# telespazio-tim/karios

Measured on AMD Instinct MI355X. Metric: Mpixels/sec (+ matched keypoints/sec), Sentinel-2 10980^2 pair, KLT + ZNCC, higher is better.
Workload: dtype u8/i32 stencils, f32 LK solve, f64 stretch + ZNCC; 1 GPU; BASELINE config 2: 4 distinct S2-sized pairs 10980x10980 u16 resident in HBM, one per step, 4 per batched submissio...; distinct_pairs_resident=4, contexts=1, klt=Laplacian k=7, maxCorners 20000, one tile, ZNCC of rows with score >= 0.4, parallelism=1 rank(s), each a stream of independent band pairs

## Files before the change

karios_amd/csrc/k_eig3.hip:

```cpp
#include <cstring>
#include <string.h>

#include "eig2_item.hpp"

namespace {

#define EIG3_STAGE 1024
#define EIG3_FLUSH_AT 384
#define EIG3_SEG 3
#define EIG3_MARGIN 12
#define EIG3_STRIDE (512 - 2 * EIG3_MARGIN)

__device__ __forceinline__ int e3_mad_lo(uint32_t a, uint32_t b, int c)
{
    int d;
    asm("v_mad_i32_i16 %0, %1, %2, %3" : "=v"(d) : "v"(a), "v"(b), "v"(c));
    return d;
}
__device__ __forceinline__ int e3_mad_hi(uint32_t a, uint32_t b, int c)
{
    int d;
    asm("v_mad_i32_i16 %0, %1, %2, %3 op_sel:[1,1,0,0]" : "=v"(d) : "v"(a), "v"(b), "v"(c));
    return d;
}
__device__ __forceinline__ uint32_t e3_pk_mad2(uint32_t a, uint32_t c)
{
    uint32_t d;
    asm("v_pk_mad_u16 %0, %1, %2, %3" : "=v"(d) : "v"(a), "s"(0x00020002u), "v"(c));
    return d;
}
__device__ __forceinline__ int e3_add_next(int w, int v)
{
    int d;
    asm("v_add_u32_dpp %0, %1, %2 wave_shl:1 row_mask:0xf bank_mask:0xf bound_ctrl:1" : "=v"(d) : "v"(v), "v"(w));
    return d;
}
__device__ __forceinline__ int e3_add_prev(int w, int v)
{
    int d;
    asm("v_add_u32_dpp %0, %1, %2 wave_shr:1 row_mask:0xf bank_mask:0xf bound_ctrl:1" : "=v"(d) : "v"(v), "v"(w));
    return d;
}
__device__ __forceinline__ int e3_next_minus(int v, int w)
{
    int d;
    asm("v_sub_u32_dpp %0, %1, %2 wave_shl:1 row_mask:0xf bank_mask:0xf bound_ctrl:1" : "=v"(d) : "v"(v), "v"(w));
    return d;
}
__device__ __forceinline__ int e3_prev_minus(int v, int w)
{
    int d;
    asm("v_sub_u32_dpp %0, %1, %2 wave_shr:1 row_mask:0xf bank_mask:0xf bound_ctrl:1" : "=v"(d) : "v"(v), "v"(w));
    return d;
}

template <class F, int... I> __device__ __forceinline__ void e3_for_impl(F &&f, std::integer_sequence<int, I...>)
{
    (f(std::integral_constant<int, I>{}), ...);
}
template <int N, class F> __device__ __forceinline__ void e3_for(F &&f) { e3_for_impl(f, std::make_integer_sequence<int, N>{}); }

template <int BLOCK>
__device__ __forceinline__ void eig3_item(const uint8_t *__restrict__ src, const uint8_t *__restrict__ mask, int H, int W, double scale2,
                                          unsigned *__restrict__ max_partial, double quality, km_scalars *sc, unsigned long long *__restrict__ keys,
                                          size_t cap, unsigned stage_cap, int wave_id, int xs, int col_lo, int col_hi, int ye0, int ye1,
                                          unsigned long long *st , int count_skips = 0)
{
    constexpr int L = BLOCK / 2, Rr = BLOCK - 1 - L;
    static_assert(L <= 7 && Rr <= 7, "the box window must stay within the two neighbouring lanes");
    const int lane = threadIdx.x & 63;
    const int c0 = xs + 8 * lane;
    const int m_first = ye0 - L, m_last = ye1 + Rr;

    uint32_t colmask[2] = {0u, 0u};
#pragma unroll
    for (int p = 0; p < 8; p++)
        if (c0 + p >= col_lo && c0 + p < col_hi) colmask[p >> 2] |= 0xffu << (8 * (p & 3));
    const uint8_t *mptr = mask ? mask : src;
    const uint32_t mask_or = mask ? 0u : 0x01010101u;

    auto load8 = [&](const uint8_t *base, int r) -> uint2 {
        const uint8_t *rowp = base + (size_t)r * W;
        uint2 v;
        __builtin_memcpy(&v, rowp + e2_opaque((unsigned)c0), 8);
        return v;
    };
    struct row4 { uint32_t q[4]; };
    auto unpack = [&](uint2 w) -> row4 {
        row4 r;
        r.q[0] = __builtin_amdgcn_perm(0u, w.x, 0x0c010c00u);
        r.q[1] = __builtin_amdgcn_perm(0u, w.x, 0x0c030c02u);
        r.q[2] = __builtin_amdgcn_perm(0u, w.y, 0x0c010c00u);
        r.q[3] = __builtin_amdgcn_perm(0u, w.y, 0x0c030c02u);
        return r;
    };
    auto derivs = [&](const row4 &r0, const row4 &r1, const row4 &r2, uint32_t (&dx)[4], uint32_t (&dy)[4]) {
        uint32_t t0[4], t1[4], m0[5], m1[5];
#pragma unroll
        for (int i = 0; i < 4; i++) {
            t0[i] = e3_pk_mad2(r1.q[i], e2u(e2s(r0.q[i]) + e2s(r2.q[i])));
            t1[i] = e2u(e2s(r2.q[i]) - e2s(r0.q[i]));
        }
        asm("s_nop 1" : "+v"(t0[0]), "+v"(t0[3]));
        const uint32_t l0 = (uint32_t)e2_lane_m1((int)t0[3]), r0n = (uint32_t)e2_lane_p1((int)t0[0]);
        const uint32_t l1 = (uint32_t)e2_lane_m1((int)t1[3]), r1n = (uint32_t)e2_lane_p1((int)t1[0]);
#pragma unroll
        for (int i = 0; i < 5; i++) {
            const uint32_t lo0 = i == 0 ? l0 : t0[i - 1], hi0 = i == 4 ? r0n : t0[i];
            const uint32_t lo1 = i == 0 ? l1 : t1[i - 1], hi1 = i == 4 ? r1n : t1[i];
            m0[i] = __builtin_amdgcn_alignbyte(hi0, lo0, 2);
            m1[i] = __builtin_amdgcn_alignbyte(hi1, lo1, 2);
        }
#pragma unroll
        for (int i = 0; i < 4; i++) {
            dx[i] = e2u(e2s(m0[i + 1]) - e2s(m0[i]));
            dy[i] = e2u(e2s(e3_pk_mad2(t1[i], m1[i])) + e2s(m1[i + 1]));
        }
    };
    int V[3][8];
#pragma unroll
    for (int q = 0; q < 3; q++)
#pragma unroll
        for (int p = 0; p < 8; p++) V[q][p] = 0;
    auto accumulate = [&](const uint32_t (&dx)[4], const uint32_t (&dy)[4], bool subtract) {
#pragma unroll
        for (int i = 0; i < 4; i++) {
            const uint32_t x = dx[i], y = dy[i];
            const uint32_t sx = subtract ? e2u(-e2s(x)) : x, sy = subtract ? e2u(-e2s(y)) : y;
            V[0][2 * i] = e3_mad_lo(x, sx, V[0][2 * i]);
            V[0][2 * i + 1] = e3_mad_hi(x, sx, V[0][2 * i + 1]);
            V[1][2 * i] = e3_mad_lo(x, sy, V[1][2 * i]);
            V[1][2 * i + 1] = e3_mad_hi(x, sy, V[1][2 * i + 1]);
            V[2][2 * i] = e3_mad_lo(y, sy, V[2][2 * i]);
            V[2][2 * i + 1] = e3_mad_hi(y, sy, V[2][2 * i + 1]);
        }
    };
    auto windows = [&](auto &&emit ) {
        auto add_ext = [&](int w, auto q_tag, auto kt) -> int {
            constexpr int q = decltype(q_tag)::value, k = decltype(kt)::value;
            if constexpr (k < 0) return e3_add_prev(w, V[q][k + 8]);
            else if constexpr (k > 7) return e3_add_next(w, V[q][k - 8]);
            else return w + V[q][k];
        };
        auto ext_minus = [&](auto q_tag, auto kt, int w) -> int {
            constexpr int q = decltype(q_tag)::value, k = decltype(kt)::value;
            if constexpr (k < 0) return e3_prev_minus(V[q][k + 8], w);
            else if constexpr (k > 7) return e3_next_minus(V[q][k - 8], w);
            else return V[q][k] - w;
        };
        int w[3];
        e3_for<3>([&](auto qt) {
            constexpr int q = decltype(qt)::value;
            if constexpr (L == 7 && Rr == 7) {
                const int T = ((V[q][0] + V[q][1]) + (V[q][2] + V[q][3])) + ((V[q][4] + V[q][5]) + (V[q][6] + V[q][7]));
                w[q] = T + e2_lane_m1(T - V[q][0]);
            } else {
                w[q] = 0;
                e3_for<BLOCK>([&](auto kt) { w[q] = add_ext(w[q], qt, std::integral_constant<int, decltype(kt)::value - L>{}); });
            }
        });
        emit(std::integral_constant<int, 0>{}, w[0], w[1], w[2]);
        e3_for<7>([&](auto pt) {
            constexpr int P = decltype(pt)::value;
            int t[3];
            e3_for<3>([&](auto qt) { t[decltype(qt)::value] = ext_minus(qt, std::integral_constant<int, P - L>{}, w[decltype(qt)::value]); });
            e3_for<3>([&](auto qt) {
                constexpr int q = decltype(qt)::value;
                w[q] = ext_minus(qt, std::integral_constant<int, P + 1 + Rr>{}, t[q]);
            });
            emit(std::integral_constant<int, P + 1>{}, w[0], w[1], w[2]);
        });
    };
    const double scale2h = scale2 * 0.5;
    auto lambda_min = [&](int sxx, int sxy, int syy) {
        const float a = (float)__dmul_rn((double)sxx, scale2h);
        const float b = (float)__dmul_rn((double)sxy, scale2);
        const float cc = (float)__dmul_rn((double)syy, scale2h);
        const float t = __fsub_rn(a, cc);
        const float sq = __fadd_rn(__fmul_rn(t, t), __fmul_rn(b, b));
        return __fsub_rn(__fadd_rn(a, cc), e2_sqrt(sq));
    };

    float best = -INFINITY;
    unsigned tie_rows = 0u;
#ifdef KM_DEV
    unsigned skip_total = 0u, skip_hit = 0u;
#endif
    unsigned cnt = 0;
    const unsigned shard = (unsigned)wave_id % KM_NSHARD;
    const size_t cap_s = cap / KM_NSHARD;
    auto flush_if = [&](unsigned threshold) {
        if (cnt <= threshold) return;
        if (cnt > stage_cap) { if (lane == 0) atomicOr(&sc->pad0, 1u); cnt = min(cnt, (unsigned)EIG3_STAGE); }
        unsigned base = 0;
        if (lane == 0) base = atomicAdd(&sc->shard_cnt[shard], cnt);
        base = __shfl(base, 0);
        for (unsigned i = lane; i < cnt; i += 64)
            if ((size_t)base + i < cap_s) keys[shard * cap_s + base + i] = st[i];
        cnt = 0;
    };
    float thr_run = 0.f;
    unsigned published = 0u, gk_seen = 0u;
    auto refresh_threshold = [&](bool global) {
        unsigned wk = best > -INFINITY ? e2_key(best) : 0u;
        for (int o = 32; o > 0; o >>= 1) wk = max(wk, (unsigned)__shfl_xor((int)wk, o));
        if (global) {
            gk_seen = __hip_atomic_load(&sc->run_max_shard[wave_id & 63], __ATOMIC_RELAXED, __HIP_MEMORY_SCOPE_AGENT);
        } else if (published == 0u && wk > gk_seen && (gk_seen == 0u || e2_unkey(wk) > e2_unkey(gk_seen) * 1.0625f)) {
            if (lane == 0) atomicMax(&sc->run_max_shard[wave_id & 63], wk);
            published = 1u;
        }
        const unsigned mk2 = max(wk, gk_seen);
        thr_run = mk2 ? (float)__dmul_rn((double)e2_unkey(mk2), quality) : 0.f;
    };

    row4 LW[3], TW[3];
    float E[3][8];
    float EM[8];
#pragma unroll
    for (int k = 0; k < 3; k++)
#pragma unroll
        for (int p = 0; p < 8; p++) E[k][p] = 0.f;
#pragma unroll
    for (int p = 0; p < 8; p++) EM[p] = -INFINITY;

    auto compute = [&](auto ph_tag, int m, uint2 mkraw, bool trail, bool out, bool cand) {
        constexpr int PH = decltype(ph_tag)::value;
        constexpr int S0 = PH, S1 = (PH + 1) % 3, S2 = (PH + 2) % 3;
        uint32_t dx[4], dy[4];
        derivs(LW[S0], LW[S1], LW[S2], dx, dy);
        accumulate(dx, dy, false);
        if (trail) {
            derivs(TW[S0], TW[S1], TW[S2], dx, dy);
            accumulate(dx, dy, true);
        }
        if (!out) return;
        const int y = m - Rr;
        constexpr int C = PH, P1 = (PH + 2) % 3, P2 = (PH + 1) % 3;
        {
            asm("s_nop 4" : "+v"(V[0][0]), "+v"(V[0][1]), "+v"(V[0][2]), "+v"(V[0][3]), "+v"(V[0][4]), "+v"(V[0][5]), "+v"(V[0][6]), "+v"(V[0][7]),
                            "+v"(V[1][0]), "+v"(V[1][1]), "+v"(V[1][2]), "+v"(V[1][3]), "+v"(V[1][4]), "+v"(V[1][5]), "+v"(V[1][6]), "+v"(V[1][7]),
                            "+v"(V[2][0]), "+v"(V[2][1]), "+v"(V[2][2]), "+v"(V[2][3]), "+v"(V[2][4]), "+v"(V[2][5]), "+v"(V[2][6]), "+v"(V[2][7]));
#ifdef KM_DEV
            if (count_skips) {
                windows([&](auto pt, int sxx, int sxy, int syy) {
                    E[C][decltype(pt)::value] = lambda_min(sxx, sxy, syy);
                    const float bound = (float)__dmul_rn((double)min(sxx, syy), scale2);
                    skip_total++;
                    skip_hit += __ballot(!(bound <= thr_run)) == 0ull ? 1u : 0u;
                });
            } else
#endif
            windows([&](auto pt, int sxx, int sxy, int syy) { E[C][decltype(pt)::value] = lambda_min(sxx, sxy, syy); });
        }
        if (cand) {
            float m3[8];
#pragma unroll
            for (int p = 0; p < 8; p++) m3[p] = fmaxf(fmaxf(E[P2][p], E[P1][p]), E[C][p]);
            const float m3l = __int_as_float(e2_lane_m1(__float_as_int(m3[7]))), m3r = __int_as_float(e2_lane_p1(__float_as_int(m3[0])));
            auto is_cand = [&](int p) {
                const float left = p == 0 ? m3l : m3[(p + 7) & 7], right = p == 7 ? m3r : m3[(p + 1) & 7];
                const float nb = fmaxf(fmaxf(left, right), m3[p]);
                return EM[p] > thr_run && EM[p] >= nb;
            };
            float selval = 0.f;
            unsigned selp = 0u, ncand = 0u;
            bool isv[8];
#pragma unroll
            for (int p = 0; p < 8; p++) {
                const bool is = isv[p] = is_cand(p);
                selval = is ? EM[p] : selval;
                selp = is ? (unsigned)p : selp;
                ncand += is ? 1u : 0u;
            }
            const unsigned rowidx = (unsigned)(y - 1) * (unsigned)W + (unsigned)c0;
            const unsigned long long multi = __ballot(ncand > 1u);
            auto append = [&](unsigned long long bal, bool mine, float v, unsigned p) {
                const unsigned slot = cnt + __builtin_amdgcn_mbcnt_hi((unsigned)(bal >> 32), __builtin_amdgcn_mbcnt_lo((unsigned)bal, 0u));
                st[min(mine ? slot : ~0u, EIG3_STAGE + (unsigned)lane)] = ((unsigned long long)__float_as_uint(v) << 32) | (unsigned long long)(rowidx + p);
                cnt += (unsigned)__popcll(bal);
            };
            if (__builtin_expect(multi == 0ull, 1)) {
                append(__ballot(ncand != 0u), ncand != 0u, selval, selp);
            } else if (__ballot(ncand > 2u) == 0ull) {
                float fval = selval;
                unsigned fp = selp;
#pragma unroll
                for (int p = 6; p >= 0; p--) {
                    fval = isv[p] ? EM[p] : fval;
                    fp = isv[p] ? (unsigned)p : fp;
                }
                append(__ballot(ncand != 0u), ncand != 0u, selval, selp);
                append(multi, ncand > 1u, fval, fp);
            } else {
                tie_rows++;
#pragma unroll
                for (int p = 0; p < 8; p++) {
                    const bool is = isv[p];
                    const unsigned long long bal = __ballot(is);
                    const unsigned slot = cnt + __builtin_amdgcn_mbcnt_hi((unsigned)(bal >> 32), __builtin_amdgcn_mbcnt_lo((unsigned)bal, 0u));
                    st[min(is ? slot : ~0u, EIG3_STAGE + (unsigned)lane)] =
                        ((unsigned long long)__float_as_uint(EM[p]) << 32) | (unsigned long long)(rowidx + (unsigned)p);
                    cnt += (unsigned)__popcll(bal);
                }
            }
        }
        const uint32_t mk[2] = {(mkraw.x | mask_or) & colmask[0], (mkraw.y | mask_or) & colmask[1]};
#pragma unroll
        for (int p = 0; p < 8; p++) {
            const bool counts = ((mk[p >> 2] >> (8 * (p & 3))) & 0xffu) != 0u;
            EM[p] = counts ? E[C][p] : -INFINITY;
            best = fmaxf(best, EM[p]);
        }
    };

    auto entering3 = [&](int m, row4 (&win)[3], auto ph_tag) {
        constexpr int PH = decltype(ph_tag)::value;
        const int r = km_reflect101(m, H);
        win[PH] = unpack(load8(src, km_reflect101(r - 1, H)));
        win[(PH + 1) % 3] = unpack(load8(src, r));
        win[(PH + 2) % 3] = unpack(load8(src, km_reflect101(r + 1, H)));
    };
    auto clamp_row = [&](int r) { return min(max(r, 0), H - 1); };
    auto general_step = [&](int m, auto ph_tag) {
        const int step = m - m_first;
        entering3(m, LW, ph_tag);
        const bool trail = step >= BLOCK;
        if (trail) entering3(m - BLOCK, TW, ph_tag);
        const bool out = step >= BLOCK - 1;
        const uint2 mkraw = load8(mptr, clamp_row(m - Rr));
        compute(ph_tag, m, mkraw, trail, out, out && (m - Rr) >= ye0 + 2);
    };
    int m = m_first;
    auto general_until = [&](int m_end, bool align3) {
        for (; m <= m_last; m++) {
            const int step = m - m_first;
            if (m > m_end && (!align3 || step % 3 == 0)) break;
            if ((step & 7) == 0) refresh_threshold(m == m_first);
            switch (step % 3) {
            case 0: general_step(m, std::integral_constant<int, 0>{}); break;
            case 1: general_step(m, std::integral_constant<int, 1>{}); break;
            default: general_step(m, std::integral_constant<int, 2>{}); break;
            }
            flush_if(EIG3_FLUSH_AT);
        }
    };
    const bool early = m_first >= 1 && BLOCK >= 5;
    const int mi_lo = early ? m_first + 1 : max(m_first + BLOCK + 1, BLOCK + 1), mi_hi = min(m_last, H - 2 - 3);
    general_until(min(mi_lo - 1, m_last), true);
    if (m <= mi_hi && m + 2 <= mi_hi) {
        uint2 ql[3], qt[3], qm[3];
#pragma unroll
        for (int k = 0; k < 3; k++) {
            ql[k] = load8(src, m + k + 1);
            qt[k] = load8(src, max(m + k - BLOCK + 1, 0));
            qm[k] = load8(mptr, max(m + k - Rr, 0));
        }
        while (m + 2 <= mi_hi && m - m_first < BLOCK + 1) {
            e3_for<3>([&](auto kt) {
                constexpr int K = decltype(kt)::value;
                const int step = m + K - m_first;
                LW[(K + 2) % 3] = unpack(ql[K]);
                TW[(K + 2) % 3] = unpack(qt[K]);
                compute(kt, m + K, qm[K], step >= BLOCK, step >= BLOCK - 1, step >= BLOCK - 1 && m + K - Rr >= ye0 + 2);
                ql[K] = load8(src, m + K + 3 + 1);
                qt[K] = load8(src, max(m + K + 3 - BLOCK + 1, 0));
                qm[K] = load8(mptr, max(m + K + 3 - Rr, 0));
            });
            m += 3;
        }
        while (m + 2 <= mi_hi) {
            flush_if(EIG3_FLUSH_AT);
            refresh_threshold(false);
            const int seg_end = min(mi_hi, m + EIG3_SEG * 3 - 1);
            for (; m + 2 <= seg_end; m += 3) {
                e3_for<3>([&](auto kt) {
                    constexpr int K = decltype(kt)::value;
                    LW[(K + 2) % 3] = unpack(ql[K]);
                    TW[(K + 2) % 3] = unpack(qt[K]);
                    compute(kt, m + K, qm[K], true, true, true);
                    ql[K] = load8(src, m + K + 3 + 1);
                    qt[K] = load8(src, m + K + 3 - BLOCK + 1);
                    qm[K] = load8(mptr, m + K + 3 - Rr);
                });
            }
        }
    }
    general_until(m_last, false);
    flush_if(0u);
    unsigned key = best > -INFINITY ? e2_key(best) : 0u;
    for (int o = 32; o > 0; o >>= 1) key = max(key, (unsigned)__shfl_xor((int)key, o));
    if (lane == 0) max_partial[wave_id] = key;
    if (lane == 0 && tie_rows) atomicAdd(&sc->tie_rows, tie_rows);
#ifdef KM_DEV
    if (lane == 0 && count_skips) { atomicAdd(&sc->skip_total, (unsigned long long)skip_total); atomicAdd(&sc->skip_hit, (unsigned long long)skip_hit); }
#endif
}

struct e3_units_args {
    const uint8_t *src[KM_UNITS_MAX], *mask[KM_UNITS_MAX];
    unsigned *max_partial[KM_UNITS_MAX];
    km_scalars *sc[KM_UNITS_MAX];
    unsigned long long *keys[KM_UNITS_MAX];
    int H[KM_UNITS_MAX], W[KM_UNITS_MAX], n_border[KM_UNITS_MAX], nstrips[KM_UNITS_MAX];
    int item0[KM_UNITS_MAX + 1];
    int n, rows2, rows3;
    int count_skips;
};
template <int BLOCK>
__global__ __launch_bounds__(256, 3) void eig3_units_kernel(e3_units_args U, double scale2, double quality, size_t cap, unsigned stage_cap2, unsigned stage_cap3)
{
    __shared__ int xs_scratch[4][3][128];
    __shared__ unsigned long long stage[4][EIG3_STAGE + 64];
    const int wv = __builtin_amdgcn_readfirstlane(threadIdx.x >> 6);
    const int total = U.item0[U.n];
    unsigned tile;
    if (!km_xcd_tile((unsigned)(total + 3) / 4u, tile)) return;
    const int wave_lin = (int)tile * 4 + wv;
    if (wave_lin >= total) return;
    int u = 0;
    while (u + 1 < U.n && wave_lin >= U.item0[u + 1]) u++;
    const int wave_id = wave_lin - U.item0[u];
    const uint8_t *src = U.src[u], *mask = U.mask[u];
    const int H = U.H[u], W = U.W[u], n_border = U.n_border[u], nstrips = U.nstrips[u];
    unsigned *max_partial = U.max_partial[u];
    km_scalars *sc = U.sc[u];
    unsigned long long *keys = U.keys[u];
    if (wave_id < n_border) {
        const int rowblock = wave_id >> 1;
        const bool right = wave_id & 1;
        constexpr int ML2 = eig2_geom<BLOCK, true>::ML;
        eig2_item<BLOCK, true>(src, mask, H, W, scale2, nullptr, max_partial, U.rows2, quality, sc, keys, cap, stage_cap2, wave_id, rowblock,
                               right ? W - EIG3_MARGIN - ML2 : -ML2, right ? W - EIG3_MARGIN : 0, right ? W : EIG3_MARGIN, &xs_scratch[wv][0][0], stage[wv]);
        return;
    }
    const int j = wave_id - n_border;
    const int rowblock = j / nstrips, strip = j - rowblock * nstrips;
    const int xs = min(strip * EIG3_STRIDE, W - 512);
    const int col_lo = EIG3_MARGIN + strip * EIG3_STRIDE, col_hi = min(col_lo + EIG3_STRIDE, W - EIG3_MARGIN);
    const int ye0 = rowblock * U.rows3, ye1 = min(H - 1, ye0 + U.rows3 + 1);
    eig3_item<BLOCK>(src, mask, H, W, scale2, max_partial, quality, sc, keys, cap, stage_cap3, wave_id, xs, col_lo, col_hi, ye0, ye1, stage[wv],
                     U.count_skips);
}

template <int BLOCK>
int launch_eig3_units(km_ctx *c, km_units &U, double scale2, double quality, bool single)
{
    e3_units_args A;
    A.n = U.n; A.rows2 = 64;
    long border_total = 0;
    for (int u = 0; u < U.n; u++) {
        A.src[u] = U.lap_ref[u]; A.mask[u] = U.mask[u]; A.sc[u] = U.sc[u]; A.keys[u] = U.keys[u];
        A.H[u] = U.H[u]; A.W[u] = U.W[u];
        A.nstrips[u] = (U.W[u] - 2 * EIG3_MARGIN + EIG3_STRIDE - 1) / EIG3_STRIDE;
        A.n_border[u] = 2 * ((U.H[u] - 2 + A.rows2 - 1) / A.rows2);
        border_total += A.n_border[u];
    }
    (void)border_total;
    int rows3 = 0;
    for (int u = 0; u < U.n; u++) {
        const int r = km_pick_rows(U.H[u] - 2, A.nstrips[u], 5, 1024L * 3 - A.n_border[u], 32, 192);
        rows3 = r > rows3 ? r : rows3;
    }
    if (!single) rows3 = std::min(std::max(rows3, 48), 96);
    if (const char *e = km_dev_env("KARIOS_HIP_EIG3_ROWS")) { const int v = atoi(e); if (v >= 8 && v <= 8192) rows3 = v; }
    A.rows3 = rows3;
    A.item0[0] = 0;
    for (int u = 0; u < U.n; u++) A.item0[u + 1] = A.item0[u] + A.n_border[u] + A.nstrips[u] * ((U.H[u] - 2 + rows3 - 1) / rows3);
    const int total = A.item0[U.n];
    unsigned *partial = (unsigned *)km_ws(c, WS_PARTIAL, ((size_t)total + 16) * sizeof(unsigned));
    if (!partial) return KM_E_NOMEM;
    for (int u = 0; u < U.n; u++) {
        A.max_partial[u] = partial + A.item0[u];
        U.eig_partial[u] = A.max_partial[u]; U.eig_npartial[u] = (unsigned)(A.item0[u + 1] - A.item0[u]);
    }
    const unsigned cap2 = c->opt_stage_cap > 0 && c->opt_stage_cap < EIG2_STAGE ? (unsigned)c->opt_stage_cap : (unsigned)EIG2_STAGE;
    const unsigned cap3 = c->opt_stage_cap > 0 && c->opt_stage_cap < EIG3_STAGE ? (unsigned)c->opt_stage_cap : (unsigned)EIG3_STAGE;
    A.count_skips = c->opt_eig3_count ? 1 : 0;
    eig3_units_kernel<BLOCK><<<km_xcd_grid((unsigned)(total + 3) / 4u), 256, 0, c->stream>>>(A, scale2, quality, U.capk, cap2, cap3);
    KM_LAUNCH_CHECK(c);
    return KM_OK;
}

__global__ __launch_bounds__(1024) void eig3_max_kernel(const unsigned *__restrict__ partial, unsigned n, unsigned *out)
{
    unsigned m = 0;
    for (unsigned i = threadIdx.x; i < n; i += 1024) m = max(m, partial[i]);
    for (int o = 32; o > 0; o >>= 1) m = max(m, (unsigned)__shfl_xor((int)m, o));
    __shared__ unsigned sh[16];
    if ((threadIdx.x & 63) == 0) sh[threadIdx.x >> 6] = m;
    __syncthreads();
    if (threadIdx.x == 0) {
        unsigned t = 0;
        for (int i = 0; i < 16; i++) t = max(t, sh[i]);
        *out = t;
    }
}

}

int k3_eig_candidates_units(km_ctx *c, km_units &U, int block, double quality)
{
    if (block < 1 || block > 15 || (block & 1) == 0 || !c->opt_eig3) return KM_E_UNSUPPORTED;
    for (int u = 0; u < U.n; u++)
        if (U.W[u] < 512 || U.H[u] < 2 * block + 8) return KM_E_UNSUPPORTED;
    const double scale = 1.0 / (4.0 * (double)block * 255.0), s2 = scale * scale;
    switch (block) {
#define KM_EIG3_CASE(B) case B: return launch_eig3_units<B>(c, U, s2, quality, false);
        KM_EIG3_CASE(1) KM_EIG3_CASE(3) KM_EIG3_CASE(5) KM_EIG3_CASE(7) KM_EIG3_CASE(9) KM_EIG3_CASE(11) KM_EIG3_CASE(13) KM_EIG3_CASE(15)
#undef KM_EIG3_CASE
    default: return KM_E_UNSUPPORTED;
    }
}

int k3_eig_candidates(km_ctx *c, const uint8_t *d_src, const uint8_t *d_mask, int H, int W, int block, double quality, km_scalars *sc,
                      unsigned long long *d_keys, size_t cap, km_eig_partials *partials)
{
    if (block < 1 || block > 15 || (block & 1) == 0) return KM_E_UNSUPPORTED;
    if (W < 512 || H < 2 * block + 8) return KM_E_UNSUPPORTED;
    const double scale = 1.0 / (4.0 * (double)block * 255.0), s2 = scale * scale;
    km_units U;
    U.n = 1; U.H[0] = H; U.W[0] = W; U.capk = cap;
    U.lap_ref[0] = const_cast<uint8_t *>(d_src); U.mask[0] = const_cast<uint8_t *>(d_mask); U.sc[0] = sc; U.keys[0] = d_keys;
    int rc;
    switch (block) {
#define KM_EIG3_CASE(B) case B: rc = launch_eig3_units<B>(c, U, s2, quality, true); break;
        KM_EIG3_CASE(1) KM_EIG3_CASE(3) KM_EIG3_CASE(5) KM_EIG3_CASE(7) KM_EIG3_CASE(9) KM_EIG3_CASE(11) KM_EIG3_CASE(13) KM_EIG3_CASE(15)
#undef KM_EIG3_CASE
    default: return KM_E_UNSUPPORTED;
    }
    if (rc) return rc;
    if (partials) {
        partials->partial = U.eig_partial[0]; partials->n = U.eig_npartial[0];
        return KM_OK;
    }
    eig3_max_kernel<<<1, 1024, 0, c->stream>>>(U.eig_partial[0], U.eig_npartial[0], &sc->max_eig_key);
    KM_LAUNCH_CHECK(c);
    return KM_OK;
}
```

Measured before the change: 160,100 Mpx/s.

## Pack leading and trailing rows into u16 pairs and accumulate with sdot2

Rows entering and leaving the sliding box window are now interleaved into one packed 16-bit pair per pixel, with the leading row in the low half and the trailing row in the high half. Derivatives for both rows are computed together, and a single v_dot2 with a sign vector (+1,-1) updates the structure-tensor sums. This replaces two separate derivative passes and pairs of mad_i32_i16 instructions, and removes the alignbyte shuffles because each pixel now sits in its own dword. The cost is twice as many registers per row window, and the pk_mad trick and 16-bit overflow behaviour now depend on the interleaving.

```diff
diff --git a/karios_amd/csrc/k_eig3.hip b/karios_amd/csrc/k_eig3.hip
--- a/karios_amd/csrc/k_eig3.hip
+++ b/karios_amd/csrc/k_eig3.hip
@@ -11,18 +11,7 @@
 #define EIG3_MARGIN 12
 #define EIG3_STRIDE (512 - 2 * EIG3_MARGIN)
 
-__device__ __forceinline__ int e3_mad_lo(uint32_t a, uint32_t b, int c)
-{
-    int d;
-    asm("v_mad_i32_i16 %0, %1, %2, %3" : "=v"(d) : "v"(a), "v"(b), "v"(c));
-    return d;
-}
-__device__ __forceinline__ int e3_mad_hi(uint32_t a, uint32_t b, int c)
-{
-    int d;
-    asm("v_mad_i32_i16 %0, %1, %2, %3 op_sel:[1,1,0,0]" : "=v"(d) : "v"(a), "v"(b), "v"(c));
-    return d;
-}
+__device__ __forceinline__ int e3_dot2(uint32_t a, uint32_t b, int c) { return __builtin_amdgcn_sdot2(e2s(a), e2s(b), c, false); }
 __device__ __forceinline__ uint32_t e3_pk_mad2(uint32_t a, uint32_t c)
 {
     uint32_t d;
@@ -85,36 +74,35 @@
         __builtin_memcpy(&v, rowp + e2_opaque((unsigned)c0), 8);
         return v;
     };
-    struct row4 { uint32_t q[4]; };
-    auto unpack = [&](uint2 w) -> row4 {
-        row4 r;
-        r.q[0] = __builtin_amdgcn_perm(0u, w.x, 0x0c010c00u);
-        r.q[1] = __builtin_amdgcn_perm(0u, w.x, 0x0c030c02u);
-        r.q[2] = __builtin_amdgcn_perm(0u, w.y, 0x0c010c00u);
-        r.q[3] = __builtin_amdgcn_perm(0u, w.y, 0x0c030c02u);
+    struct row8 { uint32_t d[8]; };
+    auto pack = [&](uint2 lead, uint2 trail) -> row8 {
+        row8 r;
+        r.d[0] = __builtin_amdgcn_perm(trail.x, lead.x, 0x0c040c00u);
+        r.d[1] = __builtin_amdgcn_perm(trail.x, lead.x, 0x0c050c01u);
+        r.d[2] = __builtin_amdgcn_perm(trail.x, lead.x, 0x0c060c02u);
+        r.d[3] = __builtin_amdgcn_perm(trail.x, lead.x, 0x0c070c03u);
+        r.d[4] = __builtin_amdgcn_perm(trail.y, lead.y, 0x0c040c00u);
+        r.d[5] = __builtin_amdgcn_perm(trail.y, lead.y, 0x0c050c01u);
+        r.d[6] = __builtin_amdgcn_perm(trail.y, lead.y, 0x0c060c02u);
+        r.d[7] = __builtin_amdgcn_perm(trail.y, lead.y, 0x0c070c03u);
         return r;
     };
-    auto derivs = [&](const row4 &r0, const row4 &r1, const row4 &r2, uint32_t (&dx)[4], uint32_t (&dy)[4]) {
-        uint32_t t0[4], t1[4], m0[5], m1[5];
-#pragma unroll
-        for (int i = 0; i < 4; i++) {
-            t0[i] = e3_pk_mad2(r1.q[i], e2u(e2s(r0.q[i]) + e2s(r2.q[i])));
-            t1[i] = e2u(e2s(r2.q[i]) - e2s(r0.q[i]));
-        }
-        asm("s_nop 1" : "+v"(t0[0]), "+v"(t0[3]));
-        const uint32_t l0 = (uint32_t)e2_lane_m1((int)t0[3]), r0n = (uint32_t)e2_lane_p1((int)t0[0]);
-        const uint32_t l1 = (uint32_t)e2_lane_m1((int)t1[3]), r1n = (uint32_t)e2_lane_p1((int)t1[0]);
-#pragma unroll
-        for (int i = 0; i < 5; i++) {
-            const uint32_t lo0 = i == 0 ? l0 : t0[i - 1], hi0 = i == 4 ? r0n : t0[i];
-            const uint32_t lo1 = i == 0 ? l1 : t1[i - 1], hi1 = i == 4 ? r1n : t1[i];
-            m0[i] = __builtin_amdgcn_alignbyte(hi0, lo0, 2);
-            m1[i] = __builtin_amdgcn_alignbyte(hi1, lo1, 2);
-        }
-#pragma unroll
-        for (int i = 0; i < 4; i++) {
-            dx[i] = e2u(e2s(m0[i + 1]) - e2s(m0[i]));
-            dy[i] = e2u(e2s(e3_pk_mad2(t1[i], m1[i])) + e2s(m1[i + 1]));
+    auto derivs = [&](const row8 &r0, const row8 &r1, const row8 &r2, uint32_t (&dx)[8], uint32_t (&dy)[8]) {
+        uint32_t t0[8], t1[8];
+#pragma unroll
+        for (int p = 0; p < 8; p++) {
+            t0[p] = e3_pk_mad2(r1.d[p], e2u(e2s(r0.d[p]) + e2s(r2.d[p])));
+            t1[p] = e2u(e2s(r2.d[p]) - e2s(r0.d[p]));
+        }
+        asm("s_nop 1" : "+v"(t0[0]), "+v"(t0[7]));
+        const uint32_t l0 = (uint32_t)e2_lane_m1((int)t0[7]), r0n = (uint32_t)e2_lane_p1((int)t0[0]);
+        const uint32_t l1 = (uint32_t)e2_lane_m1((int)t1[7]), r1n = (uint32_t)e2_lane_p1((int)t1[0]);
+#pragma unroll
+        for (int p = 0; p < 8; p++) {
+            const uint32_t lo0 = p == 0 ? l0 : t0[(p + 7) & 7], hi0 = p == 7 ? r0n : t0[(p + 1) & 7];
+            const uint32_t lo1 = p == 0 ? l1 : t1[(p + 7) & 7], hi1 = p == 7 ? r1n : t1[(p + 1) & 7];
+            dx[p] = e2u(e2s(hi0) - e2s(lo0));
+            dy[p] = e2u(e2s(e3_pk_mad2(t1[p], lo1)) + e2s(hi1));
         }
     };
     int V[3][8];
@@ -122,17 +110,13 @@
     for (int q = 0; q < 3; q++)
 #pragma unroll
         for (int p = 0; p < 8; p++) V[q][p] = 0;
-    auto accumulate = [&](const uint32_t (&dx)[4], const uint32_t (&dy)[4], bool subtract) {
-#pragma unroll
-        for (int i = 0; i < 4; i++) {
-            const uint32_t x = dx[i], y = dy[i];
-            const uint32_t sx = subtract ? e2u(-e2s(x)) : x, sy = subtract ? e2u(-e2s(y)) : y;
-            V[0][2 * i] = e3_mad_lo(x, sx, V[0][2 * i]);
-            V[0][2 * i + 1] = e3_mad_hi(x, sx, V[0][2 * i + 1]);
-            V[1][2 * i] = e3_mad_lo(x, sy, V[1][2 * i]);
-            V[1][2 * i + 1] = e3_mad_hi(x, sy, V[1][2 * i + 1]);
-            V[2][2 * i] = e3_mad_lo(y, sy, V[2][2 * i]);
-            V[2][2 * i + 1] = e3_mad_hi(y, sy, V[2][2 * i + 1]);
+    auto accumulate = [&](const uint32_t (&dx)[8], const uint32_t (&dy)[8], uint32_t sign) {
+#pragma unroll
+        for (int p = 0; p < 8; p++) {
+            const uint32_t sx = e2u(e2s(dx[p]) * e2s(sign)), sy = e2u(e2s(dy[p]) * e2s(sign));
+            V[0][p] = e3_dot2(dx[p], sx, V[0][p]);
+            V[1][p] = e3_dot2(dx[p], sy, V[1][p]);
+            V[2][p] = e3_dot2(dy[p], sy, V[2][p]);
         }
     };
     auto windows = [&](auto &&emit ) {
@@ -214,7 +198,7 @@
         thr_run = mk2 ? (float)__dmul_rn((double)e2_unkey(mk2), quality) : 0.f;
     };
 
-    row4 LW[3], TW[3];
+    row8 PW[3];
     float E[3][8];
     float EM[8];
 #pragma unroll
@@ -227,13 +211,9 @@
     auto compute = [&](auto ph_tag, int m, uint2 mkraw, bool trail, bool out, bool cand) {
         constexpr int PH = decltype(ph_tag)::value;
         constexpr int S0 = PH, S1 = (PH + 1) % 3, S2 = (PH + 2) % 3;
-        uint32_t dx[4], dy[4];
-        derivs(LW[S0], LW[S1], LW[S2], dx, dy);
-        accumulate(dx, dy, false);
-        if (trail) {
-            derivs(TW[S0], TW[S1], TW[S2], dx, dy);
-            accumulate(dx, dy, true);
-        }
+        uint32_t dx[8], dy[8];
+        derivs(PW[S0], PW[S1], PW[S2], dx, dy);
+        accumulate(dx, dy, trail ? 0xffff0001u : 0x00000001u);
         if (!out) return;
         const int y = m - Rr;
         constexpr int C = PH, P1 = (PH + 2) % 3, P2 = (PH + 1) % 3;
@@ -314,19 +294,25 @@
         }
     };
 
-    auto entering3 = [&](int m, row4 (&win)[3], auto ph_tag) {
+    auto entering3 = [&](int m, bool trail, auto ph_tag) {
         constexpr int PH = decltype(ph_tag)::value;
         const int r = km_reflect101(m, H);
-        win[PH] = unpack(load8(src, km_reflect101(r - 1, H)));
-        win[(PH + 1) % 3] = unpack(load8(src, r));
-        win[(PH + 2) % 3] = unpack(load8(src, km_reflect101(r + 1, H)));
+        uint2 t[3] = {make_uint2(0u, 0u), make_uint2(0u, 0u), make_uint2(0u, 0u)};
+        if (trail) {
+            const int rt = km_reflect101(m - BLOCK, H);
+            t[0] = load8(src, km_reflect101(rt - 1, H));
+            t[1] = load8(src, rt);
+            t[2] = load8(src, km_reflect101(rt + 1, H));
+        }
+        PW[PH] = pack(load8(src, km_reflect101(r - 1, H)), t[0]);
+        PW[(PH + 1) % 3] = pack(load8(src, r), t[1]);
+        PW[(PH + 2) % 3] = pack(load8(src, km_reflect101(r + 1, H)), t[2]);
     };
     auto clamp_row = [&](int r) { return min(max(r, 0), H - 1); };
     auto general_step = [&](int m, auto ph_tag) {
         const int step = m - m_first;
-        entering3(m, LW, ph_tag);
         const bool trail = step >= BLOCK;
-        if (trail) entering3(m - BLOCK, TW, ph_tag);
+        entering3(m, trail, ph_tag);
         const bool out = step >= BLOCK - 1;
         const uint2 mkraw = load8(mptr, clamp_row(m - Rr));
         compute(ph_tag, m, mkraw, trail, out, out && (m - Rr) >= ye0 + 2);
@@ -360,8 +346,7 @@
             e3_for<3>([&](auto kt) {
                 constexpr int K = decltype(kt)::value;
                 const int step = m + K - m_first;
-                LW[(K + 2) % 3] = unpack(ql[K]);
-                TW[(K + 2) % 3] = unpack(qt[K]);
+                PW[(K + 2) % 3] = pack(ql[K], qt[K]);
                 compute(kt, m + K, qm[K], step >= BLOCK, step >= BLOCK - 1, step >= BLOCK - 1 && m + K - Rr >= ye0 + 2);
                 ql[K] = load8(src, m + K + 3 + 1);
                 qt[K] = load8(src, max(m + K + 3 - BLOCK + 1, 0));
@@ -376,8 +361,7 @@
             for (; m + 2 <= seg_end; m += 3) {
                 e3_for<3>([&](auto kt) {
                     constexpr int K = decltype(kt)::value;
-                    LW[(K + 2) % 3] = unpack(ql[K]);
-                    TW[(K + 2) % 3] = unpack(qt[K]);
+                    PW[(K + 2) % 3] = pack(ql[K], qt[K]);
                     compute(kt, m + K, qm[K], true, true, true);
                     ql[K] = load8(src, m + K + 3 + 1);
                     qt[K] = load8(src, m + K + 3 - BLOCK + 1);
```

Measured after the change: 162,500 Mpx/s, median of 6. 1.5% higher.
